# Cuberick-Orion/Candidate-Reranking-CIR

Hardware: AMD Instinct MI355X
Metric: query-candidate triplets scored/sec at K=100 (higher is better)
Workload: dtype f16; 1 GPU; CIRR-val-style K=100 re-rank from pixels (BASELINE configs[2]): ViT-B/16 224px (197 tokens), 32-token captions, 64 queries x (100 candidates + 5 subset members) per step per GPU, skip rate 0, random-init weights; k=100, subset=5, image_size=224, residual_stream=f16

## Files before the change

### candidate_reranking_cir_amd/csrc/gemm.hip

```cpp

#include <type_traits>

#include "gemm_args.hpp"

namespace cir {

constexpr int BM = 128, BN = 128, BK = 64;
constexpr int kTileBytes = BM * BK * 2;

template <> struct Elem<float> {
    using x8 = f32x4;
};
template <typename T> struct Tile {
    static constexpr int kChunk = 16 / (int)sizeof(T);
    static constexpr int kBK = 128 / (int)sizeof(T);
};
template <typename T>
__device__ __forceinline__ void mma_frag(f32x4& acc, const typename Elem<T>::x8& w, const typename Elem<T>::x8& x) {
    if constexpr (std::is_same<T, float>::value) {
#pragma unroll
        for (int s = 0; s < 4; ++s) acc = __builtin_amdgcn_mfma_f32_16x16x4f32(w[s], x[s], acc, 0, 0, 0);
    } else {
        acc = Elem<T>::mfma16(w, x, acc);
    }
// ... 402 lines not shown
    if (ldx >= (1 << 21) || ldw >= (1 << 21)) return CIR_ESHAPE;
    if (!cir_aligned16(X) || !cir_aligned16(Wg) || !cir_aligned16(C) || !cir_aligned16(colsum) || !cir_aligned16(bias) || ldx % 8 || ldw % 8 || ldc % 8)
        return CIR_EALIGN;
    GemmArgs a;
    a.A = X; a.lda = ldx; a.sA = 0;
    a.W = Wg; a.ldw = ldw; a.sW = 0;
    a.bias = bias; a.sBias = 0;
    a.R = nullptr; a.ldr = 0; a.sR = 0;
    a.C = C; a.ldc = ldc; a.sC = 0;
    a.M = M; a.N = N; a.K = K; a.batch = 1; a.act = act; a.group_w = 1; a.dbg = 0;
    a.colsum = colsum; a.ln_eps = eps;
    if (((M + 255) / 256) * (int64_t)((N + 255) / 256) > 0x7fffffff) return CIR_ESHAPE;
    launch_gemm256(a, CIR_F16, 3, reinterpret_cast<hipStream_t>(stream));
    CIR_LAUNCH_RESULT();
}
```

### candidate_reranking_cir_amd/csrc/gemm256.hip

```cpp

#include <cstdlib>
#include <type_traits>

#include "gemm_args.hpp"

namespace cir {

#ifdef CIR_GEMM_STAMPS
__device__ unsigned long long g_stamps[2][64][8];
__device__ unsigned long long g_blk[512][4];
#define STAMP_BLK(O)                                                                                        \
    if (wave == 0 && lane == 0 && blockIdx.x < 512) {                                                       \
        unsigned long long t_, r_;                                                                          \
        asm volatile("s_memtime %0\n\ts_memrealtime %1\n\ts_waitcnt lgkmcnt(0)" : "=s"(t_), "=s"(r_) :: "memory"); \
        g_blk[blockIdx.x][O] = t_; g_blk[blockIdx.x][(O) + 1] = r_;                                         \
    }
#define STAMP(SLOT)                                                                                         \
    if (blockIdx.x == 0 && (wave == 0 || wave == 4) && lane == 0 && tile_no < 64) {                        \
        unsigned long long t_;                                                                              \
        asm volatile("s_memtime %0\n\ts_waitcnt lgkmcnt(0)" : "=s"(t_) :: "memory");                    \
        g_stamps[wave >> 2][tile_no][SLOT] = t_;                                                            \
    }
__device__ unsigned long long g_pair[2][64][8];
#define STAMP_PAIR(SLOT)                                                                                    \
// ... 2 lines not shown
        asm volatile("s_memtime %0\n\ts_waitcnt lgkmcnt(0)" : "=s"(t_) :: "memory");                    \
        g_pair[wave >> 2][tile_no][SLOT] = t_;                                                              \
    }
#else
#define STAMP(SLOT)
#define STAMP_BLK(O)
#define STAMP_PAIR(SLOT)
#endif

#define STORE_C(P, V) asm volatile("global_store_dwordx4 %0, %1, off nt\n\ts_nop 1" :: "v"(P), "v"(V) : "memory");

constexpr int T256 = 256;
constexpr int kHalf = 16384;
constexpr int kDbuf = 4 * kHalf;

template <typename T, bool OUT_F32, bool HAS_RES, typename ST = float, int ACT = -1, bool LNF = false, bool MIX = false, bool OSPL = false>
__global__ __launch_bounds__(512, 2) void gemm256_kernel(const GemmArgs a) {
    constexpr bool FAST16 = !__is_same(ST, float);
    static_assert(!(FAST16 && OUT_F32), "the stream type is written by the 16-bit epilogue");
    static_assert(!LNF || (__is_same(T, _Float16) && !OUT_F32 && !HAS_RES && !FAST16), "LNF: fp16 stream rows in, operand-type C out");
    static_assert(!MIX || (__is_same(T, _Float16) && OUT_F32 && !LNF), "MIX: split8 operand rows in, fp32 accumulators out through the fp32-layout epilogue");
    static_assert(!OSPL || (MIX && !HAS_RES), "OSPL: split8 rows out of a MIX GEMM without a residual");
    using OT = typename std::conditional<FAST16, ST, T>::type;
    using X8 = typename Elem<T>::x8;
    __shared__ __attribute__((aligned(16))) char smem[2 * kDbuf + 8 * 1024 + 4 * 4096];

    const int tid = threadIdx.x;
    const int lane = tid & 63;
    const int wave = __builtin_amdgcn_readfirstlane(tid >> 6);
    const int wr = wave >> 2, wc = wave & 3;
    const int r15 = lane & 15, g = lane >> 4;
    const int srow = lane >> 3;
    const int schunk = (lane & 7) ^ srow;
    const int nk = a.K >> 6;
    const int per_batch = a.tiles_m * a.tiles_n;
// ... 95 lines not shown
    MM4(MH, 16) MM(MH, 20) PLACE(P3) MM(MH, 21) MM(MH, 22) MM(MH, 23) MM(MH, 24) PLACE(P4) MM(MH, 25) MM(MH, 26)         \
    MM(MH, 27) MM(MH, 28) PLACE(P5) MM(MH, 29) MM(MH, 30) MM(MH, 31)
[[maybe_unused]] int sc_a = 0, sc_w = 0;
#define CAT8(X) __builtin_bit_cast(i32x8, __builtin_shufflevector((X)[0], (X)[1], 0, 1, 2, 3, 4, 5, 6, 7, 8, 9, 10, 11, 12, 13, 14, 15))
#define MF(MH, J) if constexpr (MIX) { mfma_f8_acc(acc[MH][((J) & 7) >> 1][(J) >> 3][(J) & 1], CAT8(wf[(J) >> 3][(J) & 1]), CAT8(af[((J) & 7) >> 1]), sc_w, sc_a); }
#define MF2(MH, J) MF(MH, J) MF(MH, (J) + 1)
#define MFMAS8_2(MH, P0, P1, P2, P3, P4, P5)                                                                             \
    MF2(MH, 0) MF2(MH, 2) PLACE(P0) MF2(MH, 4) MF2(MH, 6) MF2(MH, 8) PLACE(P1) MF2(MH, 10) MF2(MH, 12) MF2(MH, 14)
#define MFMAS8_6(MH, P0, P1, P2, P3, P4, P5)                                                                             \
    MF2(MH, 0) PLACE(P0) MF2(MH, 2) MF(MH, 4) PLACE(P1) MF(MH, 5) MF2(MH, 6) PLACE(P2) MF2(MH, 8) MF(MH, 10) PLACE(P3)   \
    MF(MH, 11) MF(MH, 12) PLACE(P4) MF(MH, 13) MF(MH, 14) PLACE(P5) MF(MH, 15)
[[maybe_unused]] float ssum[2] = {0.f, 0.f}, ssq[2] = {0.f, 0.f};
[[maybe_unused]] X8 sf[2];
[[maybe_unused]] const char* const s_rd = a_rd + wc * 2048;
#define READ_S(H, DB)                                                                                  \
    if constexpr (LNF) {    \
        const unsigned s0_ = (unsigned)(size_t)(lptr_t)(s_rd + (DB) * kDbuf + (H) * kHalf + c0);       \
        const unsigned s1_ = (unsigned)(size_t)(lptr_t)(s_rd + (DB) * kDbuf + (H) * kHalf + c1);       \
        __builtin_amdgcn_sched_barrier(0);                                                             \
        asm volatile("ds_read_b128 %0, %2\n\tds_read_b128 %1, %3" : "=&v"(sf[0]), "=&v"(sf[1]) : "v"(s0_), "v"(s1_)); \
        __builtin_amdgcn_sched_barrier(0);                                                             \
    }
#define ST1(MH, D)                                                                                     \
    { const unsigned d_ = __builtin_bit_cast(u32x4, sf[(D) >> 2])[(D) & 3];                            \
      asm volatile("v_fma_mix_f32 %0, %2, 1.0, %0 op_sel:[0,0,0] op_sel_hi:[1,0,0]\n\tv_fma_mix_f32 %1, %2, %2, %1 op_sel:[0,0,0] op_sel_hi:[1,1,0]\n\t" \
                   "v_fma_mix_f32 %0, %2, 1.0, %0 op_sel:[1,0,0] op_sel_hi:[1,0,0]\n\tv_fma_mix_f32 %1, %2, %2, %1 op_sel:[1,1,0] op_sel_hi:[1,1,0]" \
                   : "+v"(ssum[MH]), "+v"(ssq[MH]) : "v"(d_)); }
#define STATS(MH, NY)             \
    if constexpr (LNF) {                                                                               \
        __builtin_amdgcn_sched_barrier(0);                                                             \
        asm volatile("s_waitcnt lgkmcnt(%0)" :: "n"(NY) : "memory");                                   \
        ST1(MH, 0) ST1(MH, 1) ST1(MH, 2) ST1(MH, 3) ST1(MH, 4) ST1(MH, 5) ST1(MH, 6) ST1(MH, 7)        \
        __builtin_amdgcn_sched_barrier(0);                                                             \
    }
#define COMPUTE(KIND, MH, NDMA, P0, P1, P2, P3, P4, P5) \
    SYNC();                                      \
    __builtin_amdgcn_s_setprio(1);               \
    MFMAS##KIND##_##NDMA(MH, P0, P1, P2, P3, P4, P5)     \
    __builtin_amdgcn_s_setprio(0);               \
    SYNC();
#define WAIT_N(N) asm volatile("s_waitcnt vmcnt(%0)" :: "n"(N) : "memory");
#define WAIT_PRO(N) if (!skip) { WAIT_N(N) }
#ifdef CIR_GEMM_STAMPS
#define WAIT_ABB() if (!(skip && (a.dbg & 0x800))) { WAIT_N(2) }
#define WAIT_A1() if (!(skip && (a.dbg & 0x400))) { WAIT_N(6) }
#else
#define WAIT_ABB() WAIT_N(2)
#define WAIT_A1() WAIT_N(6)
#endif

    static_assert(!HAS_RES || OUT_F32 || FAST16, "the residual is added in a row layout of the epilogue");

    char* const bias_slot = smem + 2 * kDbuf + wave * 1024;
#define ISSUE_BIAS()                                                                                                   \
    if constexpr (LNF) {                                                                                               \
        int ln_ = lane;                                                                                                \
        asm volatile("" : "+v"(ln_));    \
        int nm4_ = __builtin_amdgcn_readfirstlane(a.N - 4);                                                            \
        asm volatile("" : "+s"(nm4_));        \
        if (ln_ < 32) {                                                                                                \
            const int bn = min(n0 + wc * 64 + (ln_ & 15) * 4, nm4_);                                                   \
            const float* src_ = (ln_ & 16) ? a.colsum : a.bias;                                                        \
            __builtin_amdgcn_global_load_lds((gptr_t)(src_ + bn), (lptr_t)(bias_slot), 16, 0, 0);                      \
        }                                                                                                              \
    } else if (a.bias != nullptr) {                                                                                    \
        int bn = n0 + lane * 4;                                                                                        \
        bn = bn + 4 <= a.N ? bn : a.N - 4;             \
        __builtin_amdgcn_global_load_lds((gptr_t)(a.bias + z * a.sBias + bn), (lptr_t)(bias_slot), 16, 0, 0);         \
    }

    int t = blockIdx.x;
#ifdef CIR_GEMM_STAMPS
    for (int i = 0, n = (a.dbg & 0xff) * ((blockIdx.x >> 3) & 3); i < n; ++i) __builtin_amdgcn_s_sleep(127);
#endif
    STAMP_BLK(0)
    adopt(coords(t));
    ISSUE_PROLOGUE()
    ISSUE_BIAS()
    int pending_stores = 0;
    [[maybe_unused]] int tile_no = 0;

    for (;;) {
        const int64_t cm0 = m0;
        const int cn0 = n0, cz = z;
        const int tn = t + (int)gridDim.x;
        const bool more = tn < ntiles;
        Coords nx = coords(more ? tn : t);
        A_nx = nx.A; W_nx = nx.W;
        stream = false;
        STAMP(0)
        if (pending_stores == 0) asm volatile("s_waitcnt vmcnt(0)" ::: "memory");
        else if (pending_stores == 16) asm volatile("s_waitcnt vmcnt(16)" ::: "memory");
        else asm volatile("s_waitcnt vmcnt(32)" ::: "memory");
// ... 29 lines not shown
            for (int mh = 0; mh < 2; ++mh)
#pragma unroll
                for (int mi = 0; mi < 4; ++mi)
#pragma unroll
                    for (int nh = 0; nh < 2; ++nh) {
                        asm volatile("" : "+v"(acc[mh][mi][nh][0]), "+v"(acc[mh][mi][nh][1]));
                    }
        }
        STAMP(2)
        SYNC();
        if (wr == 1) { SYNC(); }
        stream = more && nx.interior && rel_interior;
        STAMP(3)

#define PUBLISH_STATS()                                                                                                      \
        if constexpr (LNF) {                                                                                                 \
            const float inv_k = 1.0f / (float)a.K;                                                                           \
            int lp_ = lane;                                                                                                  \
            asm volatile("" : "+v"(lp_));                                                                                    \
            const unsigned xw = (unsigned)(size_t)(lptr_t)(bias_slot) + 512 + (lp_ & 15) * 8;                                \
            _Pragma("unroll") for (int mh = 0; mh < 2; ++mh) {                                                               \
                float sx = ssum[mh], sq = ssq[mh], t0, t1;                                                                   \
                asm volatile("v_mov_b32 %2, %0\n\tv_mov_b32 %3, %1\n\ts_nop 1\n\tv_permlane32_swap_b32 %0, %2\n\tv_permlane32_swap_b32 %1, %3\n\ts_nop 1\n\t" \
                             "v_add_f32 %0, %0, %2\n\tv_add_f32 %1, %1, %3\n\tv_mov_b32 %2, %0\n\tv_mov_b32 %3, %1\n\ts_nop 1\n\t"           \
                             "v_permlane16_swap_b32 %0, %2\n\tv_permlane16_swap_b32 %1, %3\n\ts_nop 1\n\tv_add_f32 %0, %0, %2\n\tv_add_f32 %1, %1, %3" \
                             : "+v"(sx), "+v"(sq), "=&v"(t0), "=&v"(t1));                                                    \
                const float mean = sx * inv_k;                                                                               \
                const float var = fmaxf(fmaf(sq, inv_k, -mean * mean), 0.f);                                                 \
                const float rstd = __builtin_amdgcn_rsqf(var + a.ln_eps);    \
                const f32x2 st = {rstd, -rstd * mean};                                                                       \
                if (lp_ < 16) asm volatile("ds_write_b64 %0, %1" :: "v"(xw + mh * 128), "v"(st) : "memory");                 \
// ... 73 lines not shown
        [[maybe_unused]] RV rres[RD][4];
#define LOAD_RES(PS)                                                                                                         \
        if constexpr (HAS_RES) {                                                                                             \
            const int prow_ = ((PS) / (NPASS / 2)) * 128 + wr * 64 + ((PS) % (NPASS / 2)) * ROWS;                            \
            _Pragma("unroll") for (int j = 0; j < 4; ++j) {                                                                  \
                const int64_t m = cm0 + prow_ + j * (64 / LPR) + rr;                                                         \
                rres[(PS) % RD][j] = (full || (m < a.M && ncol + REL <= a.N))                                                \
                    ? *reinterpret_cast<const RV*>(reinterpret_cast<const ST*>(a.R) + cz * a.sR + m * a.ldr + ncol) : RV{};  \
            }                                                                                                                \
        }
        _Pragma("unroll") for (int p = 0; p < RD; ++p) { LOAD_RES(p) }
        __builtin_amdgcn_sched_barrier(0);
        [[maybe_unused]] float lb[2][8], ls[2][8], lal[2][4], lnm[2][4];
        if constexpr (LNF) {
            const unsigned baddr = (unsigned)(size_t)(lptr_t)(bias_slot) + (unsigned)(ge * 32);
            const unsigned xr = (unsigned)(size_t)(lptr_t)(smem + 2 * kDbuf + wr * 4096 + 512) + r15e * 8;
            f32x4 b00, b01, b10, b11, s00, s01, s10, s11;
            f32x2 t00, t01, t02, t03, t10, t11, t12, t13;
            asm volatile("ds_read_b128 %0, %8\n\tds_read_b128 %1, %8 offset:16\n\tds_read_b128 %2, %8 offset:128\n\t"
                         "ds_read_b128 %3, %8 offset:144\n\tds_read_b128 %4, %8 offset:256\n\tds_read_b128 %5, %8 offset:272\n\t"
                         "ds_read_b128 %6, %8 offset:384\n\tds_read_b128 %7, %8 offset:400\n\ts_waitcnt lgkmcnt(0)"
                         : "=&v"(b00), "=&v"(b01), "=&v"(b10), "=&v"(b11), "=&v"(s00), "=&v"(s01), "=&v"(s10), "=&v"(s11)
                         : "v"(baddr) : "memory");
            asm volatile("ds_read_b64 %0, %8\n\tds_read_b64 %1, %8 offset:1024\n\tds_read_b64 %2, %8 offset:2048\n\t"
                         "ds_read_b64 %3, %8 offset:3072\n\tds_read_b64 %4, %8 offset:128\n\tds_read_b64 %5, %8 offset:1152\n\t"
                         "ds_read_b64 %6, %8 offset:2176\n\tds_read_b64 %7, %8 offset:3200\n\ts_waitcnt lgkmcnt(0)"
                         : "=&v"(t00), "=&v"(t01), "=&v"(t02), "=&v"(t03), "=&v"(t10), "=&v"(t11), "=&v"(t12), "=&v"(t13)
                         : "v"(xr) : "memory");
#pragma unroll
            for (int q = 0; q < 4; ++q) {
                lb[0][q] = b00[q]; lb[0][4 + q] = b01[q]; lb[1][q] = b10[q]; lb[1][4 + q] = b11[q];
                ls[0][q] = s00[q]; ls[0][4 + q] = s01[q]; ls[1][q] = s10[q]; ls[1][4 + q] = s11[q];
            }
            lal[0][0] = t00.x; lnm[0][0] = t00.y; lal[0][1] = t01.x; lnm[0][1] = t01.y; lal[0][2] = t02.x; lnm[0][2] = t02.y; lal[0][3] = t03.x; lnm[0][3] = t03.y;
            lal[1][0] = t10.x; lnm[1][0] = t10.y; lal[1][1] = t11.x; lnm[1][1] = t11.y; lal[1][2] = t12.x; lnm[1][2] = t12.y; lal[1][3] = t13.x; lnm[1][3] = t13.y;
        }
        __builtin_amdgcn_sched_barrier(0);

        if (more) {
            const bool streamed = stream;
            stream = false;
            adopt(nx);
            if (!streamed) { ISSUE_PROLOGUE() }
            ISSUE_BIAS()
        }
        __builtin_amdgcn_sched_barrier(0);
        if constexpr (LNF) {
#pragma unroll
            for (int mh = 0; mh < 2; ++mh)
#pragma unroll
                for (int mi = 0; mi < 4; ++mi)
#pragma unroll
                    for (int nh = 0; nh < 2; ++nh)
#pragma unroll
                        for (int ni = 0; ni < 2; ++ni)
#pragma unroll
                            for (int jp = 0; jp < 2; ++jp) {
                                const int q = ni * 4 + jp * 2;
                                const f32x2 al2 = {lal[mh][mi], lal[mh][mi]}, nm2 = {lnm[mh][mi], lnm[mh][mi]};
// ... 145 lines not shown
                        if constexpr (OUT_F32) cp = reinterpret_cast<u32x4*>(reinterpret_cast<float*>(a.C) + cz * a.sC + m * a.ldc + ncol);
                        else cp = reinterpret_cast<u32x4*>(reinterpret_cast<OT*>(a.C) + cz * a.sC + m * a.ldc + ncol);
                        STORE_C(cp, dd[j])
                    }
                }
                if (ps + RD < NPASS) { LOAD_RES(ps + RD) }
                if (ps + 1 < NPASS) { WRITE_STAGE() }
            }
#undef PRODUCE
#undef LOAD_RES
#undef WRITE_STAGE
        }
        pending_stores = full ? (OUT_F32 ? 32 : 16) : 0;
        STAMP(7)
        ++tile_no;
        if (!more) break;
        t = tn;
    }
    asm volatile("s_waitcnt vmcnt(0)" ::: "memory");
    STAMP_BLK(2)
#undef ISSUE_BIAS
#undef ISSUE_A
#undef ISSUE_B
#undef ISSUE_A1
#undef LDS_DMA
#undef PIECE_A
#undef PIECE_B
#undef ISSUE_B1
#undef ISSUE_PROLOGUE
#undef READ_A
// ... 51 lines not shown
}

void launch_gemm256(const GemmArgs& a_in, int in_dtype, int out_kind, hipStream_t s) {
    GemmArgs a = a_in;
    const dim3 grid = plan256(a), block(512);
#ifdef CIR_GEMM_STAMPS
    if (const char* e = getenv("CIR_DBG")) a.dbg = (int)strtol(e, nullptr, 0);
#endif
    const bool res = a.R != nullptr;
#define CIR_LAUNCH256(...) hipLaunchKernelGGL((gemm256_kernel<__VA_ARGS__>), grid, block, 0, s, a)
    if (out_kind == 3) {
        if (a.act == CIR_ACT_GELU) CIR_LAUNCH256(_Float16, false, false, float, CIR_ACT_GELU, true);
        else CIR_LAUNCH256(_Float16, false, false, float, CIR_ACT_NONE, true);
        return;
    }
#define CIR_DISPATCH256(T)                                                                                                     \
    if (out_kind == 1) {                                                                                                       \
        if (a.act == CIR_ACT_NONE) { if (res) CIR_LAUNCH256(T, true, true, float, CIR_ACT_NONE); else CIR_LAUNCH256(T, true, false, float, CIR_ACT_NONE); } \
        else { if (res) CIR_LAUNCH256(T, true, true); else CIR_LAUNCH256(T, true, false); }                                    \
    }                                                                                                                          \
    else if (out_kind == 2) {                                                                                                  \
        if (a.act == CIR_ACT_NONE) { if (res) CIR_LAUNCH256(T, false, true, _Float16, CIR_ACT_NONE); else CIR_LAUNCH256(T, false, false, _Float16, CIR_ACT_NONE); } \
        else { if (res) CIR_LAUNCH256(T, false, true, _Float16); else CIR_LAUNCH256(T, false, false, _Float16); }              \
    } else if (a.act == CIR_ACT_NONE) CIR_LAUNCH256(T, false, false, float, CIR_ACT_NONE);                                    \
    else if (a.act == CIR_ACT_GELU) CIR_LAUNCH256(T, false, false, float, CIR_ACT_GELU);                                      \
    else CIR_LAUNCH256(T, false, false);
    if (in_dtype == CIR_BF16) { CIR_DISPATCH256(__bf16) } else { CIR_DISPATCH256(_Float16) }
#undef CIR_DISPATCH256
#undef CIR_LAUNCH256
}
// ... 20 lines not shown
```

### candidate_reranking_cir_amd/csrc/gemm_args.hpp

```cpp
#pragma once
#include "common.hpp"

namespace cir {

struct GemmArgs {
    const void* A; int64_t lda, sA;
    const void* W; int64_t ldw, sW;
    const float* bias; int64_t sBias;
    const void* R; int64_t ldr, sR;
    void* C; int64_t ldc, sC;
    int64_t M; int N, K, batch, act, tiles_m, tiles_n;
    int dbg;
    int group_w;
    const float* colsum = nullptr;
    float ln_eps = 0.f;
    int k16 = 0;
    int sc_a1 = 0, sc_w1 = 0, sc_a2 = 0, sc_w2 = 0;
    int n_logical = 0;
};

typedef __attribute__((address_space(1))) const void* gptr_t;
typedef __attribute__((address_space(3))) void* lptr_t;

void launch_gemm256(const GemmArgs& a, int in_dtype, int out_kind, hipStream_t s);
void launch_gemm256_split8(const GemmArgs& a, int out_split, hipStream_t s);

}
```

### candidate_reranking_cir_amd/engine.py

```python
from __future__ import annotations

import warnings
import weakref
from typing import Dict, NamedTuple, Optional, Tuple

import torch

from . import ops
from .config import BertGeometry, VitGeometry

SD = Dict[str, torch.Tensor]

LN_FOLD_DEFAULT = 1


def _w16(t: torch.Tensor, dtype, device) -> torch.Tensor:
    return t.detach().to(device=device, dtype=torch.float32).to(dtype).contiguous()


def _f32(t: torch.Tensor, device) -> torch.Tensor:
    return t.detach().to(device=device, dtype=torch.float32).contiguous()


def _mark_split(mode: int, layers, *extra):
    mark = ops.split_weight8 if mode == 8 else ops.split_weight
    for ly in layers:
        for k, v in ly.items():
            if k.startswith("w") and torch.is_tensor(v) and v.dtype == torch.float32 and v.dim() >= 2:
# ... 51 lines not shown
        self.b_patch = _f32(sd[p + "patch_embed.proj.bias"], device)
        self.cls = _f32(sd[p + "cls_token"].reshape(d), device)
        self.pos = _f32(sd[p + "pos_embed"].reshape(-1, d), device)
        self.blocks = []
        for i in range(geo.depth):
            b = f"{p}blocks.{i}."
            self.blocks.append(dict(
                g1=_f32(sd[b + "norm1.weight"], device), b1=_f32(sd[b + "norm1.bias"], device),
                wqkv=_w16(sd[b + "attn.qkv.weight"], dtype, device), bqkv=_f32(sd[b + "attn.qkv.bias"], device),
                wo=_w16(sd[b + "attn.proj.weight"], dtype, device), bo=_f32(sd[b + "attn.proj.bias"], device),
                g2=_f32(sd[b + "norm2.weight"], device), b2=_f32(sd[b + "norm2.bias"], device),
                w1=_w16(sd[b + "mlp.fc1.weight"], dtype, device), c1=_f32(sd[b + "mlp.fc1.bias"], device),
                w2=_w16(sd[b + "mlp.fc2.weight"], dtype, device), c2=_f32(sd[b + "mlp.fc2.bias"], device)))
        self.gf, self.bf = _f32(sd[p + "norm.weight"], device), _f32(sd[p + "norm.bias"], device)
        self.ln_fold = 0
        if dtype == torch.float16 and self.stream_dtype == torch.float16 and d % 128 == 0:
            self.ln_fold = LN_FOLD_DEFAULT
            for i, blk in enumerate(self.blocks):
                b = f"{p}blocks.{i}."
                blk["qkv_f"] = ops.ln_fold_pack(sd[b + "attn.qkv.weight"].to(device), sd[b + "attn.qkv.bias"].to(device), blk["g1"], blk["b1"])
                if self.ln_fold >= 2:
                    blk["fc1_f"] = ops.ln_fold_pack(sd[b + "mlp.fc1.weight"].to(device), sd[b + "mlp.fc1.bias"].to(device), blk["g2"], blk["b2"])

    def forward(self, image: Optional[torch.Tensor], want32: bool = False, chunk: int = 4096, out32: Optional[torch.Tensor] = None,
                out16: Optional[torch.Tensor] = None, patches: Optional[torch.Tensor] = None):
        if patches is not None:
            return self._forward_patches(patches, want32, chunk, out32, out16)
        geo, dt = self.geo, self.dtype
        bsz, d, n = image.shape[0], geo.width, geo.num_tokens
        if bsz > chunk:
            n_parts = -(-bsz // chunk)
            size = -(-bsz // n_parts)
            y16 = torch.empty((bsz, n, d), dtype=dt, device=image.device) if out16 is None else out16
            if dt == torch.float32 and want32 and out32 is None:
                y32 = y16
            else:
                y32 = (torch.empty((bsz, n, d), dtype=torch.float32, device=image.device) if out32 is None else out32) if want32 else None
# ... 21 lines not shown
            y32 = y16
        else:
            y32 = (torch.empty((bsz, n, d), dtype=torch.float32, device=patches.device) if out32 is None else out32) if want32 else None
        for i in range(0, bsz, size):
            self._encode(patches[i * p:(i + size) * p], min(size, bsz - i), want32, None if y32 is None else y32[i:i + size], y16[i:i + size])
        return y32, y16

    def _encode(self, patches: torch.Tensor, bsz: int, want32: bool, out32: Optional[torch.Tensor], out16: Optional[torch.Tensor]):
        geo, dt = self.geo, self.dtype
        d, n = geo.width, geo.num_tokens
        scale = 64 ** -0.5
        sdt = self.stream_dtype
        proj = ops.gemm(patches, self.w_patch, self.b_patch, out_dtype=sdt)
        x = ops.vit_assemble(proj, self.cls, self.pos, bsz).view(bsz * n, d)
        ctx = torch.empty((bsz, n, d), dtype=dt, device=x.device)
        for blk in self.blocks:
            if self.ln_fold >= 1:
                qkv = ops.gemm_ln(x, *blk["qkv_f"], geo.layer_norm_eps).view(bsz, n, 3, d)
            else:
                _, xb = _ln(x, blk["g1"], blk["b1"], geo.layer_norm_eps, dt, sdt, need_stream=False)
                qkv = ops.gemm(xb, blk["wqkv"], blk["bqkv"]).view(bsz, n, 3, d)
            ops.attention(qkv[:, :, 0].unsqueeze(1), qkv[:, :, 1].unsqueeze(1), qkv[:, :, 2].unsqueeze(1),
                          ctx.unsqueeze(1), scale)
            ops.gemm(ctx.view(bsz * n, d), blk["wo"], blk["bo"], residual=x, out_dtype=sdt, out=x)
            if self.ln_fold >= 2 and "fc1_f" in blk:
                f = ops.gemm_ln(x, *blk["fc1_f"], geo.layer_norm_eps, act=ops.ACT_GELU)
            else:
                _, xb = _ln(x, blk["g2"], blk["b2"], geo.layer_norm_eps, dt, sdt, need_stream=False)
                f = ops.gemm(xb, blk["w1"], blk["c1"], act=ops.ACT_GELU)
            ops.gemm(f, blk["w2"], blk["c2"], residual=x, out_dtype=sdt, out=x)
        if dt == torch.float32:
            o = out16 if out16 is not None else out32
            y32, _ = ops.layernorm(x, self.gf, self.bf, geo.layer_norm_eps, want32=True, dtype16=None, stream_dtype=torch.float32,
                                   out32=None if o is None else o.view(bsz * n, d))
            if out16 is not None and out32 is not None and out32.data_ptr() != out16.data_ptr():
                out32.copy_(out16)
            return (y32.view(bsz, n, d) if want32 else None), y32.view(bsz, n, d)
        y32, y16 = ops.layernorm(x, self.gf, self.bf, geo.layer_norm_eps, want32=want32, dtype16=dt, stream_dtype=torch.float32,
                                 out32=None if (out32 is None or not want32) else out32.view(bsz * n, d),
                                 out16=None if out16 is None else out16.view(bsz * n, d))
# ... 412 lines not shown
```

### candidate_reranking_cir_amd/lib.py

```python
from __future__ import annotations

import ctypes
import os
from ctypes import c_uint64, c_char_p, c_float, c_int, c_int64, c_void_p

_HERE = os.path.dirname(os.path.abspath(__file__))
LIB_PATH = os.environ.get("CIR_LIB", os.path.join(_HERE, "libcirrank.so"))

CIR_BF16, CIR_F16, CIR_F32 = 0, 1, 2
TUNE_GEMM_TILE, TUNE_GEMM_GROUP_W, TUNE_ATTN_SHARED_MAX = 0, 1, 2
ACT_NONE, ACT_GELU, ACT_RELU = 0, 1, 2

class WgradDesc(ctypes.Structure):
    _fields_ = [("dy", c_void_p), ("ldy", c_int64), ("x", c_void_p), ("ldx", c_int64), ("dw", c_void_p), ("ldw", c_int64), ("rows", c_int64),
                ("N", c_int), ("K", c_int), ("splits", c_int)]


SIGNATURES = {
    "cir_version": (c_int, []),
    "cir_strerror": (c_char_p, [c_int]),
    "cir_set_tuning": (c_int, [c_int, c_int]),
    "cir_gemm_bias_act": (c_int, [c_void_p, c_int64, c_int64, c_void_p, c_int64, c_int64, c_void_p, c_int64,
                                  c_void_p, c_int, c_int64, c_int64, c_void_p, c_int64, c_int64,
                                  c_int64, c_int, c_int, c_int, c_int, c_int, c_int, c_void_p]),
    "cir_gemm_ln_bias_act": (c_int, [c_void_p, c_int64, c_void_p, c_int64, c_void_p, c_void_p, c_void_p, c_int64,
                                     c_int64, c_int, c_int, c_float, c_int, c_int, c_void_p]),
    "cir_split16": (c_int, [c_void_p, c_int64, c_void_p, c_void_p, c_void_p, c_int64, c_int64, c_int, c_int, c_void_p]),
    "cir_split8": (c_int, [c_void_p, c_int64, c_void_p, c_int64, c_int64, c_int, c_int, c_void_p]),
    "cir_gemm_split8": (c_int, [c_void_p, c_int64, c_int64, c_void_p, c_int64, c_int64, c_void_p, c_int64, c_void_p, c_int64, c_int64,
                                c_void_p, c_int64, c_int64, c_int64, c_int, c_int, c_int, c_int, c_int, c_int, c_int, c_void_p]),
    "cir_layernorm_split8": (c_int, [c_void_p, c_int64, c_void_p, c_int64, c_void_p, c_void_p, c_int64, c_void_p, c_int64, c_void_p, c_int64, c_int64,
                                     c_int64, c_int, c_int, c_float, c_void_p]),
    "cir_layernorm": (c_int, [c_void_p, c_int, c_int64, c_void_p, c_int64, c_void_p, c_void_p, c_int64, c_void_p, c_int, c_void_p,
                              c_int64, c_int64, c_int, c_int, c_float, c_int, c_void_p]),
    "cir_attention": (c_int, [c_void_p, c_int64, c_int64, c_int64, c_void_p, c_int64, c_int64, c_int64,
                              c_void_p, c_int64, c_int64, c_int64, c_void_p, c_int64, c_int64, c_void_p,
                              c_void_p, c_int64, c_int64, c_int64,
                              c_int, c_int, c_int, c_int, c_int, c_float, c_int, c_void_p]),
    "cir_attention_split8": (c_int, [c_void_p, c_int64, c_int64, c_int64, c_void_p, c_int64, c_int64, c_int64, c_void_p, c_int64, c_int64, c_int64,
                                     c_void_p, c_int64, c_int64, c_void_p, c_int64, c_int64, c_int64, c_int, c_int, c_int, c_int, c_int, c_float, c_void_p]),
    "cir_cls_cross_attention": (c_int, [c_void_p, c_int64, c_void_p, c_void_p, c_void_p, c_int, c_int, c_int, c_float, c_int, c_void_p]),
# ... 112 lines not shown
```

### candidate_reranking_cir_amd/ops.py

```python
from __future__ import annotations

from typing import Optional

import torch

from . import lib as _lib
from .lib import ACT_GELU, ACT_NONE, ACT_RELU, CIR_BF16, CIR_F16, CIR_F32

_DT = {torch.bfloat16: CIR_BF16, torch.float16: CIR_F16, torch.float32: CIR_F32}


PROFILE_GEMM = None
PROFILE_ATTN = None


def gemm_kernel_name(m: int, n: int, k: int, nb: int, has_residual: bool, act: int, out_dtype, in_dtype: torch.dtype, tile: int = 0,
                     res_dtype=None, lda: int = 0, ldw: int = 0, form: str = "gemm") -> str:
    if form == "ln":
        return f"cir::gemm256_kernel<_Float16,false,false,float,{act},true>"
    split8 = form == "split8"
    if in_dtype == torch.float32 and not split8:
        return "cir::gemm_kernel<float,1>"
    if isinstance(out_dtype, bool):
        out_dtype = torch.float32 if out_dtype else in_dtype
    t = "__bf16" if in_dtype == torch.bfloat16 else "_Float16"
    stream16 = out_dtype == torch.float16 and (in_dtype != torch.float16 or (has_residual and res_dtype == torch.float16))
    kind = 1 if out_dtype == torch.float32 else (2 if stream16 else 0)
    nblk256 = -(-m // 256) * -(-n // 256) * nb
    use256 = n >= 256 and nblk256 >= 192
    can256 = split8 or (not (has_residual and (act != ACT_NONE or kind == 0)) and k % 128 == 0)
    if tile == 128:
        use256 = False
    elif tile == 256:
        use256 = True
# ... 241 lines not shown
    assert colsum.dtype == torch.float32 and bias.dtype == torch.float32 and colsum.shape == (n,) and bias.shape == (n,)
    if out is None:
        out = torch.empty((m, n), dtype=torch.float16, device=x.device)
    assert out.shape == (m, n) and out.dtype == torch.float16 and out.stride(1) == 1
    ev = _events() if PROFILE_GEMM is not None else None
    code = _lib.load().cir_gemm_ln_bias_act(x.data_ptr(), x.stride(0), wg.data_ptr(), wg.stride(0), colsum.data_ptr(), bias.data_ptr(),
                                            out.data_ptr(), out.stride(0), m, n, k, float(eps), act, CIR_F16, _stream())
    if ev is not None:
        ev[1].record()
        PROFILE_GEMM.append((2.0 * m * n * k, *ev, float((m * k + n * k + m * n) * 2 + n * 8),
                             gemm_kernel_name(m, n, k, 1, False, act, torch.float16, torch.float16, form="ln")))
    _lib.check(code, "cir_gemm_ln_bias_act")
    return out


def _ln_views(x: torch.Tensor, gamma: torch.Tensor, residual: Optional[torch.Tensor], dtypes):
    x3 = x if x.dim() == 3 else x.unsqueeze(0)
    nb = max(x3.shape[0], gamma.shape[0] if gamma.dim() == 2 else 1, (residual.shape[0] if residual is not None and residual.dim() == 3 else 1))
    rows, cols = x3.shape[1], x3.shape[2]
    assert x3.dtype in dtypes and x3.stride(2) == 1 and x3.stride(1) == cols
    sx = x3.stride(0) if x3.shape[0] > 1 else 0
    sr = 0
    if residual is not None:
        r3 = residual if residual.dim() == 3 else residual.unsqueeze(0)
        assert r3.dtype == x3.dtype and r3.stride(2) == 1 and r3.stride(1) == cols
        sr = r3.stride(0) if r3.shape[0] > 1 else 0
    sg = gamma.stride(0) if gamma.dim() == 2 else 0
    return x3, nb, rows, cols, ((nb, rows) if (x.dim() == 3 or nb > 1) else (rows,)), sx, sr, sg


# ... 296 lines not shown
```

### include/cirrank.h

```cpp
#ifndef CIRRANK_H
#define CIRRANK_H

#include <stdint.h>

#ifdef __cplusplus
extern "C" {
#endif

#define CIR_ABI_VERSION 15

enum { CIR_BF16 = 0, CIR_F16 = 1, CIR_F32 = 2 };
enum { CIR_ACT_NONE = 0, CIR_ACT_GELU = 1, CIR_ACT_RELU = 2 };
enum {
    CIR_OK = 0,
    CIR_EINVAL = -1,
    CIR_ESHAPE = -2,
    CIR_EALIGN = -3,
    CIR_EDTYPE = -4
};

int cir_version(void);
const char* cir_strerror(int code);

enum { CIR_TUNE_GEMM_TILE = 0, CIR_TUNE_GEMM_GROUP_W = 1, CIR_TUNE_ATTN_SHARED_MAX = 2 };
int cir_set_tuning(int knob, int value);

int cir_gemm_bias_act(const void* A, int64_t lda, int64_t strideA,
                      const void* W, int64_t ldw, int64_t strideW,
                      const float* bias, int64_t strideBias,
                      const void* residual, int res_dtype, int64_t ldr, int64_t strideR,
                      void* C, int64_t ldc, int64_t strideC,
                      int64_t M, int N, int K, int batch,
                      int act, int in_dtype, int out_dtype, void* stream);

int cir_gemm_ln_bias_act(const void* X, int64_t ldx, const void* Wg, int64_t ldw, const float* colsum, const float* bias,
                         void* C, int64_t ldc, int64_t M, int N, int K, float eps, int act, int dtype, void* stream);

int cir_split16(const float* x, int64_t ldx, void* hi, void* lo, void* hi2, int64_t ldo, int64_t rows, int cols, int act, void* stream);

int cir_split8(const float* x, int64_t ldx, void* out, int64_t ldo_bytes, int64_t rows, int cols, int act, void* stream);

int cir_attention_split8(const float* q, int64_t q_s1, int64_t q_s0, int64_t q_rs, const float* k, int64_t k_s1, int64_t k_s0, int64_t k_rs,
                         const float* v, int64_t v_s1, int64_t v_s0, int64_t v_rs, const float* mask, int64_t m_s1, int64_t m_s0,
                         void* out, int64_t o_s1_bytes, int64_t o_s0_bytes, int64_t o_rs_bytes, int B1, int B0, int H, int Lq, int Lk,
                         float scale, void* stream);

int cir_layernorm_split8(const float* x, int64_t strideX, const float* residual, int64_t strideR, const float* gamma, const float* beta,
                         int64_t strideG, float* y_stream, int64_t strideY, void* y_split, int64_t ld_split_bytes, int64_t stride_split_bytes,
                         int64_t rows, int cols, int batch, float eps, void* stream);

int cir_gemm_split8(const void* A, int64_t lda_bytes, int64_t strideA_bytes, const void* W, int64_t ldw_bytes, int64_t strideW_bytes,
// ... 145 lines not shown
```

Before: 18330 triplets/s.

## Split LN-folded GEMM into stats-producing head launch and stats-reusing rest launch

Adds a split variant of the LayerNorm-folded GEMM. A first launch computes a narrow column slice while also accumulating per-row mean and variance, and writes those statistics to a global buffer. A second launch covers the remaining columns and reads the stored stats through the bias LDS slot, so it skips the in-loop statistics reduction. This is meant to take the per-row LN stats work off the critical path of most tiles. The cost is an extra kernel launch and an ordering dependency between the two launches, and it is enabled by default for QKV and optionally for fc1.

Result: no change. 18420 triplets/s (median of 6 runs) (+0.5%).

```diff
diff --git a/candidate_reranking_cir_amd/csrc/gemm.hip b/candidate_reranking_cir_amd/csrc/gemm.hip
--- a/candidate_reranking_cir_amd/csrc/gemm.hip
+++ b/candidate_reranking_cir_amd/csrc/gemm.hip
@@ -440,3 +440,41 @@
     launch_gemm256(a, CIR_F16, 3, reinterpret_cast<hipStream_t>(stream));
     CIR_LAUNCH_RESULT();
 }
+
+extern "C" int cir_gemm_ln_split(const void* X, int64_t ldx, const void* Wg, int64_t ldw, const float* colsum, const float* bias,
+                                 void* C, int64_t ldc, int64_t M, int N, int K, float eps, int act, int dtype, int head_cols,
+                                 void* stats, int64_t stats_bytes, int parts, void* stream) {
+    using namespace cir;
+    CIR_CHECK_PTR(X); CIR_CHECK_PTR(Wg); CIR_CHECK_PTR(colsum); CIR_CHECK_PTR(bias); CIR_CHECK_PTR(C); CIR_CHECK_PTR(stats);
+    if (M <= 0 || N <= 0 || K <= 0 || !(eps > 0.f)) return CIR_EINVAL;
+    if (dtype != CIR_F16) return CIR_EDTYPE;
+    if (act != CIR_ACT_NONE && act != CIR_ACT_GELU) return CIR_EINVAL;
+    if (head_cols <= 0 || parts < 1 || parts > 3) return CIR_EINVAL;
+    if (K % 128 != 0 || N % 16 != 0 || N < 64 || head_cols % 256 != 0) return CIR_ESHAPE;
+    if (N > head_cols && N - head_cols < 64) return CIR_ESHAPE;
+    if (ldx >= (1 << 21) || ldw >= (1 << 21)) return CIR_ESHAPE;
+    const int64_t tiles_m = (M + 255) / 256;
+    if (tiles_m * (int64_t)((N + 255) / 256) > 0x7fffffff) return CIR_ESHAPE;
+    if (stats_bytes < tiles_m * 2048) return CIR_ESHAPE;
+    if (!cir_aligned16(X) || !cir_aligned16(Wg) || !cir_aligned16(C) || !cir_aligned16(colsum) || !cir_aligned16(bias) || !cir_aligned16(stats) ||
+        ldx % 8 || ldw % 8 || ldc % 8)
+        return CIR_EALIGN;
+    GemmArgs a;
+    a.A = X; a.lda = ldx; a.sA = 0;
+    a.W = Wg; a.ldw = ldw; a.sW = 0;
+    a.bias = bias; a.sBias = 0;
+    a.R = nullptr; a.ldr = 0; a.sR = 0;
+    a.C = C; a.ldc = ldc; a.sC = 0;
+    a.M = M; a.N = N < head_cols ? N : head_cols; a.K = K; a.batch = 1; a.act = act; a.group_w = 1; a.dbg = 0;
+    a.colsum = colsum; a.ln_eps = eps; a.stats = stats;
+    hipStream_t s = reinterpret_cast<hipStream_t>(stream);
+    if (parts & 1) launch_gemm256(a, CIR_F16, 4, s);
+    if ((parts & 2) && N > head_cols) {
+        a.W = reinterpret_cast<const _Float16*>(Wg) + (int64_t)head_cols * ldw;
+        a.bias = bias + head_cols; a.colsum = colsum + head_cols;
+        a.C = reinterpret_cast<_Float16*>(C) + head_cols;
+        a.N = N - head_cols;
+        launch_gemm256(a, CIR_F16, 5, s);
+    }
+    CIR_LAUNCH_RESULT();
+}
diff --git a/candidate_reranking_cir_amd/csrc/gemm256.hip b/candidate_reranking_cir_amd/csrc/gemm256.hip
--- a/candidate_reranking_cir_amd/csrc/gemm256.hip
+++ b/candidate_reranking_cir_amd/csrc/gemm256.hip
@@ -40,11 +40,13 @@
 constexpr int kHalf = 16384;
 constexpr int kDbuf = 4 * kHalf;
 
-template <typename T, bool OUT_F32, bool HAS_RES, typename ST = float, int ACT = -1, bool LNF = false, bool MIX = false, bool OSPL = false>
+template <typename T, bool OUT_F32, bool HAS_RES, typename ST = float, int ACT = -1, bool LNF = false, bool MIX = false, bool OSPL = false, int LNS = 0>
 __global__ __launch_bounds__(512, 2) void gemm256_kernel(const GemmArgs a) {
     constexpr bool FAST16 = !__is_same(ST, float);
     static_assert(!(FAST16 && OUT_F32), "the stream type is written by the 16-bit epilogue");
     static_assert(!LNF || (__is_same(T, _Float16) && !OUT_F32 && !HAS_RES && !FAST16), "LNF: fp16 stream rows in, operand-type C out");
+    static_assert(LNS == 0 || (LNF && LNS <= 2), "LNS: the two launches of a split LNF GEMM");
+    constexpr bool LSTAT = LNF && LNS != 2;
     static_assert(!MIX || (__is_same(T, _Float16) && OUT_F32 && !LNF), "MIX: split8 operand rows in, fp32 accumulators out through the fp32-layout epilogue");
     static_assert(!OSPL || (MIX && !HAS_RES), "OSPL: split8 rows out of a MIX GEMM without a residual");
     using OT = typename std::conditional<FAST16, ST, T>::type;
@@ -170,7 +172,7 @@
 [[maybe_unused]] X8 sf[2];
 [[maybe_unused]] const char* const s_rd = a_rd + wc * 2048;
 #define READ_S(H, DB)                                                                                  \
-    if constexpr (LNF) {    \
+    if constexpr (LSTAT) {    \
         const unsigned s0_ = (unsigned)(size_t)(lptr_t)(s_rd + (DB) * kDbuf + (H) * kHalf + c0);       \
         const unsigned s1_ = (unsigned)(size_t)(lptr_t)(s_rd + (DB) * kDbuf + (H) * kHalf + c1);       \
         __builtin_amdgcn_sched_barrier(0);                                                             \
@@ -183,7 +185,7 @@
                    "v_fma_mix_f32 %0, %2, 1.0, %0 op_sel:[1,0,0] op_sel_hi:[1,0,0]\n\tv_fma_mix_f32 %1, %2, %2, %1 op_sel:[1,1,0] op_sel_hi:[1,1,0]" \
                    : "+v"(ssum[MH]), "+v"(ssq[MH]) : "v"(d_)); }
 #define STATS(MH, NY)             \
-    if constexpr (LNF) {                                                                               \
+    if constexpr (LSTAT) {                                                                             \
         __builtin_amdgcn_sched_barrier(0);                                                             \
         asm volatile("s_waitcnt lgkmcnt(%0)" :: "n"(NY) : "memory");                                   \
         ST1(MH, 0) ST1(MH, 1) ST1(MH, 2) ST1(MH, 3) ST1(MH, 4) ST1(MH, 5) ST1(MH, 6) ST1(MH, 7)        \
@@ -208,18 +210,26 @@
     static_assert(!HAS_RES || OUT_F32 || FAST16, "the residual is added in a row layout of the epilogue");
 
     char* const bias_slot = smem + 2 * kDbuf + wave * 1024;
-#define ISSUE_BIAS()                                                                                                   \
+#define ISSUE_BIAS(PG)                                                                                                 \
     if constexpr (LNF) {                                                                                               \
         int ln_ = lane;                                                                                                \
         asm volatile("" : "+v"(ln_));    \
         int nm4_ = __builtin_amdgcn_readfirstlane(a.N - 4);                                                            \
         asm volatile("" : "+s"(nm4_));        \
-        if (ln_ < 32) {                                                                                                \
+        if constexpr (LNS == 2) {                                                                                      \
+            if (ln_ < 32 || (ln_ >> 4) == 2 + (PG)) {                                                                  \
+                const int bn = min(n0 + wc * 64 + (ln_ & 15) * 4, nm4_);                                               \
+                const float* src_ = (ln_ & 16) ? a.colsum : a.bias;                                                    \
+                src_ += bn;                                                                                            \
+                if (ln_ >= 32) src_ = reinterpret_cast<const float*>(a.stats) + ((m0 >> 8) * 512 + wave * 64 + (ln_ & 15) * 4); \
+                __builtin_amdgcn_global_load_lds((gptr_t)(src_), (lptr_t)(bias_slot), 16, 0, 0);                       \
+            }                                                                                                          \
+        } else if (ln_ < 32) {                                                                                         \
             const int bn = min(n0 + wc * 64 + (ln_ & 15) * 4, nm4_);                                                   \
             const float* src_ = (ln_ & 16) ? a.colsum : a.bias;                                                        \
             __builtin_amdgcn_global_load_lds((gptr_t)(src_ + bn), (lptr_t)(bias_slot), 16, 0, 0);                      \
         }                                                                                                              \
-    } else if (a.bias != nullptr) {                                                                                    \
+    } else if (a.bias != nullptr) {                                                                                  \
         int bn = n0 + lane * 4;                                                                                        \
         bn = bn + 4 <= a.N ? bn : a.N - 4;             \
         __builtin_amdgcn_global_load_lds((gptr_t)(a.bias + z * a.sBias + bn), (lptr_t)(bias_slot), 16, 0, 0);         \
@@ -232,7 +242,8 @@
     STAMP_BLK(0)
     adopt(coords(t));
     ISSUE_PROLOGUE()
-    ISSUE_BIAS()
+    [[maybe_unused]] int page = 0;
+    ISSUE_BIAS(page)
     int pending_stores = 0;
     [[maybe_unused]] int tile_no = 0;
 
@@ -292,7 +303,7 @@
         STAMP(3)
 
 #define PUBLISH_STATS()                                                                                                      \
-        if constexpr (LNF) {                                                                                                 \
+        if constexpr (LSTAT) {                                                                                                 \
             const float inv_k = 1.0f / (float)a.K;                                                                           \
             int lp_ = lane;                                                                                                  \
             asm volatile("" : "+v"(lp_));                                                                                    \
@@ -396,7 +407,7 @@
         [[maybe_unused]] float lb[2][8], ls[2][8], lal[2][4], lnm[2][4];
         if constexpr (LNF) {
             const unsigned baddr = (unsigned)(size_t)(lptr_t)(bias_slot) + (unsigned)(ge * 32);
-            const unsigned xr = (unsigned)(size_t)(lptr_t)(smem + 2 * kDbuf + wr * 4096 + 512) + r15e * 8;
+            const unsigned xr = (unsigned)(size_t)(lptr_t)(smem + 2 * kDbuf + wr * 4096 + 512) + r15e * 8 + (LNS == 2 ? page * 256 : 0);
             f32x4 b00, b01, b10, b11, s00, s01, s10, s11;
             f32x2 t00, t01, t02, t03, t10, t11, t12, t13;
             asm volatile("ds_read_b128 %0, %8\n\tds_read_b128 %1, %8 offset:16\n\tds_read_b128 %2, %8 offset:128\n\t"
@@ -416,6 +427,16 @@
             }
             lal[0][0] = t00.x; lnm[0][0] = t00.y; lal[0][1] = t01.x; lnm[0][1] = t01.y; lal[0][2] = t02.x; lnm[0][2] = t02.y; lal[0][3] = t03.x; lnm[0][3] = t03.y;
             lal[1][0] = t10.x; lnm[1][0] = t10.y; lal[1][1] = t11.x; lnm[1][1] = t11.y; lal[1][2] = t12.x; lnm[1][2] = t12.y; lal[1][3] = t13.x; lnm[1][3] = t13.y;
+            if constexpr (LNS == 1) {
+                if (lane_e < 32) {
+                    const unsigned pa_ = (unsigned)(size_t)(lptr_t)(bias_slot) + 512 + lane_e * 8;
+                    const unsigned vo_ = lane_e * 8;
+                    const char* const ib_ = reinterpret_cast<const char*>(a.stats) + ((cm0 >> 8) * 2048 + wave * 256);
+                    u32x2 pv_;
+                    asm volatile("ds_read_b64 %0, %1\n\ts_waitcnt lgkmcnt(0)" : "=&v"(pv_) : "v"(pa_) : "memory");
+                    asm volatile("global_store_dwordx2 %0, %1, %2\n\ts_nop 1" :: "v"(vo_), "v"(pv_), "s"(ib_) : "memory");
+                }
+            }
         }
         __builtin_amdgcn_sched_barrier(0);
 
@@ -424,7 +445,7 @@
             stream = false;
             adopt(nx);
             if (!streamed) { ISSUE_PROLOGUE() }
-            ISSUE_BIAS()
+            ISSUE_BIAS(page ^ 1)
         }
         __builtin_amdgcn_sched_barrier(0);
         if constexpr (LNF) {
@@ -600,6 +621,7 @@
         pending_stores = full ? (OUT_F32 ? 32 : 16) : 0;
         STAMP(7)
         ++tile_no;
+        if constexpr (LNS == 2) page ^= 1;
         if (!more) break;
         t = tn;
     }
@@ -681,6 +703,16 @@
         else CIR_LAUNCH256(_Float16, false, false, float, CIR_ACT_NONE, true);
         return;
     }
+    if (out_kind == 4 || out_kind == 5) {
+        if (out_kind == 4) {
+            if (a.act == CIR_ACT_GELU) CIR_LAUNCH256(_Float16, false, false, float, CIR_ACT_GELU, true, false, false, 1);
+            else CIR_LAUNCH256(_Float16, false, false, float, CIR_ACT_NONE, true, false, false, 1);
+        } else {
+            if (a.act == CIR_ACT_GELU) CIR_LAUNCH256(_Float16, false, false, float, CIR_ACT_GELU, true, false, false, 2);
+            else CIR_LAUNCH256(_Float16, false, false, float, CIR_ACT_NONE, true, false, false, 2);
+        }
+        return;
+    }
 #define CIR_DISPATCH256(T)                                                                                                     \
     if (out_kind == 1) {                                                                                                       \
         if (a.act == CIR_ACT_NONE) { if (res) CIR_LAUNCH256(T, true, true, float, CIR_ACT_NONE); else CIR_LAUNCH256(T, true, false, float, CIR_ACT_NONE); } \
diff --git a/candidate_reranking_cir_amd/csrc/gemm_args.hpp b/candidate_reranking_cir_amd/csrc/gemm_args.hpp
--- a/candidate_reranking_cir_amd/csrc/gemm_args.hpp
+++ b/candidate_reranking_cir_amd/csrc/gemm_args.hpp
@@ -14,6 +14,7 @@
     int group_w;
     const float* colsum = nullptr;
     float ln_eps = 0.f;
+    void* stats = nullptr;
     int k16 = 0;
     int sc_a1 = 0, sc_w1 = 0, sc_a2 = 0, sc_w2 = 0;
     int n_logical = 0;
diff --git a/candidate_reranking_cir_amd/engine.py b/candidate_reranking_cir_amd/engine.py
--- a/candidate_reranking_cir_amd/engine.py
+++ b/candidate_reranking_cir_amd/engine.py
@@ -1,5 +1,6 @@
 from __future__ import annotations
 
+import os
 import warnings
 import weakref
 from typing import Dict, NamedTuple, Optional, Tuple
@@ -12,6 +13,8 @@
 SD = Dict[str, torch.Tensor]
 
 LN_FOLD_DEFAULT = 1
+LN_SPLIT_DEFAULT = 1
+LN_SPLIT_FC1_HEAD_COLS = 512
 
 
 def _w16(t: torch.Tensor, dtype, device) -> torch.Tensor:
@@ -93,13 +96,27 @@
                 w2=_w16(sd[b + "mlp.fc2.weight"], dtype, device), c2=_f32(sd[b + "mlp.fc2.bias"], device)))
         self.gf, self.bf = _f32(sd[p + "norm.weight"], device), _f32(sd[p + "norm.bias"], device)
         self.ln_fold = 0
+        self.ln_split = 0
+        self._fc1_src = None
         if dtype == torch.float16 and self.stream_dtype == torch.float16 and d % 128 == 0:
             self.ln_fold = LN_FOLD_DEFAULT
+            self.ln_split = LN_SPLIT_DEFAULT
+            if os.environ.get("CIR_VIT_LNSPLIT") in ("0", "1", "2"):
+                self.ln_split = int(os.environ["CIR_VIT_LNSPLIT"])
+            self._fc1_src = [(sd[f"{p}blocks.{i}.mlp.fc1.weight"], sd[f"{p}blocks.{i}.mlp.fc1.bias"]) for i in range(geo.depth)]
             for i, blk in enumerate(self.blocks):
                 b = f"{p}blocks.{i}."
                 blk["qkv_f"] = ops.ln_fold_pack(sd[b + "attn.qkv.weight"].to(device), sd[b + "attn.qkv.bias"].to(device), blk["g1"], blk["b1"])
-                if self.ln_fold >= 2:
-                    blk["fc1_f"] = ops.ln_fold_pack(sd[b + "mlp.fc1.weight"].to(device), sd[b + "mlp.fc1.bias"].to(device), blk["g2"], blk["b2"])
+            if self.ln_fold >= 2 or self.ln_split >= 2:
+                self.pack_fc1()
+
+    def pack_fc1(self) -> bool:
+        if self._fc1_src is None:
+            return False
+        for blk, (w, b) in zip(self.blocks, self._fc1_src):
+            if "fc1_f" not in blk:
+                blk["fc1_f"] = ops.ln_fold_pack(w.to(self.device), b.to(self.device), blk["g2"], blk["b2"])
+        return True
 
     def forward(self, image: Optional[torch.Tensor], want32: bool = False, chunk: int = 4096, out32: Optional[torch.Tensor] = None,
                 out16: Optional[torch.Tensor] = None, patches: Optional[torch.Tensor] = None):
@@ -151,8 +168,13 @@
         proj = ops.gemm(patches, self.w_patch, self.b_patch, out_dtype=sdt)
         x = ops.vit_assemble(proj, self.cls, self.pos, bsz).view(bsz * n, d)
         ctx = torch.empty((bsz, n, d), dtype=dt, device=x.device)
+        fold = self.ln_fold if "qkv_f" in self.blocks[0] else 0
+        split = self.ln_split if fold >= 1 else 0
+        fold_fc1 = (fold >= 2 and "fc1_f" in self.blocks[0]) or (split >= 2 and self.pack_fc1())
         for blk in self.blocks:
-            if self.ln_fold >= 1:
+            if split >= 1:
+                qkv = ops.gemm_ln_split(x, *blk["qkv_f"], geo.layer_norm_eps).view(bsz, n, 3, d)
+            elif fold >= 1:
                 qkv = ops.gemm_ln(x, *blk["qkv_f"], geo.layer_norm_eps).view(bsz, n, 3, d)
             else:
                 _, xb = _ln(x, blk["g1"], blk["b1"], geo.layer_norm_eps, dt, sdt, need_stream=False)
@@ -160,7 +182,9 @@
             ops.attention(qkv[:, :, 0].unsqueeze(1), qkv[:, :, 1].unsqueeze(1), qkv[:, :, 2].unsqueeze(1),
                           ctx.unsqueeze(1), scale)
             ops.gemm(ctx.view(bsz * n, d), blk["wo"], blk["bo"], residual=x, out_dtype=sdt, out=x)
-            if self.ln_fold >= 2 and "fc1_f" in blk:
+            if fold_fc1 and split >= 2:
+                f = ops.gemm_ln_split(x, *blk["fc1_f"], geo.layer_norm_eps, act=ops.ACT_GELU, head_cols=LN_SPLIT_FC1_HEAD_COLS)
+            elif fold_fc1:
                 f = ops.gemm_ln(x, *blk["fc1_f"], geo.layer_norm_eps, act=ops.ACT_GELU)
             else:
                 _, xb = _ln(x, blk["g2"], blk["b2"], geo.layer_norm_eps, dt, sdt, need_stream=False)
diff --git a/candidate_reranking_cir_amd/lib.py b/candidate_reranking_cir_amd/lib.py
--- a/candidate_reranking_cir_amd/lib.py
+++ b/candidate_reranking_cir_amd/lib.py
@@ -25,6 +25,8 @@
                                   c_int64, c_int, c_int, c_int, c_int, c_int, c_int, c_void_p]),
     "cir_gemm_ln_bias_act": (c_int, [c_void_p, c_int64, c_void_p, c_int64, c_void_p, c_void_p, c_void_p, c_int64,
                                      c_int64, c_int, c_int, c_float, c_int, c_int, c_void_p]),
+    "cir_gemm_ln_split": (c_int, [c_void_p, c_int64, c_void_p, c_int64, c_void_p, c_void_p, c_void_p, c_int64,
+                                  c_int64, c_int, c_int, c_float, c_int, c_int, c_int, c_void_p, c_int64, c_int, c_void_p]),
     "cir_split16": (c_int, [c_void_p, c_int64, c_void_p, c_void_p, c_void_p, c_int64, c_int64, c_int, c_int, c_void_p]),
     "cir_split8": (c_int, [c_void_p, c_int64, c_void_p, c_int64, c_int64, c_int, c_int, c_void_p]),
     "cir_gemm_split8": (c_int, [c_void_p, c_int64, c_int64, c_void_p, c_int64, c_int64, c_void_p, c_int64, c_void_p, c_int64, c_int64,
diff --git a/candidate_reranking_cir_amd/ops.py b/candidate_reranking_cir_amd/ops.py
--- a/candidate_reranking_cir_amd/ops.py
+++ b/candidate_reranking_cir_amd/ops.py
@@ -18,6 +18,8 @@
                      res_dtype=None, lda: int = 0, ldw: int = 0, form: str = "gemm") -> str:
     if form == "ln":
         return f"cir::gemm256_kernel<_Float16,false,false,float,{act},true>"
+    if form in ("ln_head", "ln_rest"):
+        return f"cir::gemm256_kernel<_Float16,false,false,float,{act},true,false,false,{1 if form == 'ln_head' else 2}>"
     split8 = form == "split8"
     if in_dtype == torch.float32 and not split8:
         return "cir::gemm_kernel<float,1>"
@@ -289,6 +291,45 @@
     return out
 
 
+LN_SPLIT_HEAD_COLS = 256
+
+
+def gemm_ln_split(x: torch.Tensor, wg: torch.Tensor, colsum: torch.Tensor, bias: torch.Tensor, eps: float, act: int = ACT_NONE,
+                  out: Optional[torch.Tensor] = None, head_cols: int = LN_SPLIT_HEAD_COLS, stats: Optional[torch.Tensor] = None) -> torch.Tensor:
+    _need_cuda(x, wg, colsum, bias, out, stats)
+    m, k = x.shape
+    n = wg.shape[0]
+    assert x.dtype == torch.float16 and wg.dtype == torch.float16 and x.stride(1) == 1 and wg.stride(1) == 1 and wg.shape[1] == k
+    assert colsum.dtype == torch.float32 and bias.dtype == torch.float32 and colsum.shape == (n,) and bias.shape == (n,)
+    if out is None:
+        out = torch.empty((m, n), dtype=torch.float16, device=x.device)
+    assert out.shape == (m, n) and out.dtype == torch.float16 and out.stride(1) == 1
+    if stats is None:
+        stats = torch.empty((-(-m // 256) * 2048,), dtype=torch.uint8, device=x.device)
+    assert stats.dtype == torch.uint8 and stats.dim() == 1 and stats.stride(0) == 1
+    fn = _lib.load().cir_gemm_ln_split
+
+    def call(parts):
+        return fn(x.data_ptr(), x.stride(0), wg.data_ptr(), wg.stride(0), colsum.data_ptr(), bias.data_ptr(), out.data_ptr(), out.stride(0),
+                  m, n, k, float(eps), act, CIR_F16, head_cols, stats.data_ptr(), stats.numel(), parts, _stream())
+
+    if PROFILE_GEMM is None:
+        code = call(3)
+    else:
+        nh = min(n, max(head_cols, 0))
+        code = 0
+        for parts, cols, form in ((1, nh, "ln_head"), (2, n - nh, "ln_rest")):
+            if cols <= 0 or code != 0:
+                continue
+            ev = _events()
+            code = call(parts)
+            ev[1].record()
+            PROFILE_GEMM.append((2.0 * m * cols * k, *ev, float((m * k + cols * k + m * cols) * 2 + cols * 8 + -(-m // 256) * 2048),
+                                 gemm_kernel_name(m, cols, k, 1, False, act, torch.float16, torch.float16, form=form)))
+    _lib.check(code, "cir_gemm_ln_split")
+    return out
+
+
 def _ln_views(x: torch.Tensor, gamma: torch.Tensor, residual: Optional[torch.Tensor], dtypes):
     x3 = x if x.dim() == 3 else x.unsqueeze(0)
     nb = max(x3.shape[0], gamma.shape[0] if gamma.dim() == 2 else 1, (residual.shape[0] if residual is not None and residual.dim() == 3 else 1))
diff --git a/include/cirrank.h b/include/cirrank.h
--- a/include/cirrank.h
+++ b/include/cirrank.h
@@ -35,6 +35,10 @@
 
 int cir_gemm_ln_bias_act(const void* X, int64_t ldx, const void* Wg, int64_t ldw, const float* colsum, const float* bias,
                          void* C, int64_t ldc, int64_t M, int N, int K, float eps, int act, int dtype, void* stream);
+
+int cir_gemm_ln_split(const void* X, int64_t ldx, const void* Wg, int64_t ldw, const float* colsum, const float* bias,
+                      void* C, int64_t ldc, int64_t M, int N, int K, float eps, int act, int dtype, int head_cols,
+                      void* stats, int64_t stats_bytes, int parts, void* stream);
 
 int cir_split16(const float* x, int64_t ldx, void* hi, void* lo, void* hi2, int64_t ldo, int64_t rows, int cols, int act, void* stream);
 
```
